# smann95/mpmc

Hardware: AMD Instinct MI355X
Metric: MC steps/sec (polarizable, 4096 atoms) (higher is better)
Workload: dtype f64; 1 GPU; PCN-61 cell + 416 BSSP H2, 4096 atoms (2016 frozen), polarizable, Jacobi x4, rc 8 A, FH4; energy() incremental (bit-identical to full); n_atoms=4096, n_polarizable=3264, n_atoms_final=4096, n_polarizable_final=3264, walkers=1, parallelism=1 independent walkers, 1 per GPU, collective=none (single walker, no launcher), rccl_ranks=1

## Files before the change

### include/mpmc_hip.h

```cpp
#ifndef MPMC_HIP_H
#define MPMC_HIP_H

#include <stddef.h>
#include <stdint.h>

#ifdef __cplusplus
extern "C" {
#endif

#define MPMC_HIP_ABI_VERSION 1

typedef struct mpmc_hip_ctx mpmc_hip_ctx;
typedef struct mpmc_hip_comm mpmc_hip_comm;

typedef struct mpmc_hip_params {
    double temperature;
    int rd_only;
    int rd_lrc;
    int feynman_hibbs;
    int feynman_hibbs_order;
    int ewald_alpha_set;
    double ewald_alpha;
    int ewald_kmax;
    int polarization;
    double polar_damp;
    int polar_max_iter;
    double polar_precision;
    double polar_gamma;
    int polar_gs;
    int polar_gs_ranked;
    int polar_sor;
    int polar_esor;
    int polar_palmo;
    int polar_rrms;
    int polar_zodid;
    int polar_wolf;
    double polar_wolf_alpha;
    int polar_ewald;
    int polar_ewald_alpha_set;
    double polar_ewald_alpha;
    int wolf;
} mpmc_hip_params;

typedef struct mpmc_hip_result {
    double energy;
    double rd_energy;
    double coulombic_energy;
    double polarization_energy;
    double es_real, es_recip, es_self;
    double dipole_rrms;
    double volume, cutoff, ewald_alpha, polar_ewald_alpha;
    int polar_iterations;
    int iter_success;
    int n_atoms;
    int status;
} mpmc_hip_result;

typedef struct mpmc_hip_timings {
    float pair_ms;
    float recip_ms;
    float field_ms;
    float amatrix_ms;
    float sweep_ms;
    float palmo_ms;
    float other_ms;
    float total_ms;
    int sweep_count;
    int amatrix_count;
    int graph_steps;
    float event_pair_ms;
    int event_pair_count;
    int spec_rank_redos;
    int resident_calls;
    int resident_fallbacks;
} mpmc_hip_timings;

const char *mpmc_hip_last_error(void);
int mpmc_hip_abi_version(void);
int mpmc_hip_device_count(void);

int mpmc_hip_create(mpmc_hip_ctx **ctx, int device, int max_atoms);
void mpmc_hip_destroy(mpmc_hip_ctx *ctx);

int mpmc_hip_set_option(mpmc_hip_ctx *ctx, const char *name, int value);

void mpmc_hip_default_params(mpmc_hip_params *p);
int mpmc_hip_set_params(mpmc_hip_ctx *ctx, const mpmc_hip_params *p);

int mpmc_hip_set_box(mpmc_hip_ctx *ctx, const double basis[9], double pbc_cutoff);

int mpmc_hip_scale_box(mpmc_hip_ctx *ctx, const double basis[9], double pbc_cutoff,
                       int n_molecules, const double *delta );

int mpmc_hip_upload(mpmc_hip_ctx *ctx, int n, const double *x, const double *y, const double *z,
                    const double *charge, const double *polarizability, const double *epsilon,
                    const double *sigma, const double *mass, const int *molecule, const uint8_t *frozen);

typedef struct mpmc_hip_disp_params {
    int disp_expansion;
    int damp_dispersion;
    int extrapolate_disp_coeffs;
    int schmidt_mixing;
} mpmc_hip_disp_params;

int mpmc_hip_set_dispersion(mpmc_hip_ctx *ctx, const mpmc_hip_disp_params *p, int n, const double *c6, const double *c8,
                            const double *c10);

int mpmc_hip_set_axilrod_teller(mpmc_hip_ctx *ctx, int enable, int n, const double *c9);
int mpmc_hip_get_three_body_energy(mpmc_hip_ctx *ctx, double *out);

int mpmc_hip_set_rd_crystal(mpmc_hip_ctx *ctx, int order);

int mpmc_hip_update_atoms(mpmc_hip_ctx *ctx, int first, int count, const double *x, const double *y,
                          const double *z);

int mpmc_hip_insert_molecule(mpmc_hip_ctx *ctx, int count, const double *x, const double *y, const double *z,
                             const double *charge, const double *polarizability, const double *epsilon,
                             const double *sigma, const double *mass, int frozen, int *first_slot);
int mpmc_hip_remove_molecule(mpmc_hip_ctx *ctx, int first_slot, int count);
int mpmc_hip_set_sweep_order(mpmc_hip_ctx *ctx, int count, const int *slots);
int mpmc_hip_slot_count(mpmc_hip_ctx *ctx);

int mpmc_hip_energy(mpmc_hip_ctx *ctx, mpmc_hip_result *out);

int mpmc_hip_energy_begin(mpmc_hip_ctx *ctx);
int mpmc_hip_energy_end(mpmc_hip_ctx *ctx, mpmc_hip_result *out);

// ... 25 lines not shown
```

### mpmc_amd/csrc/engine.hip

```cpp
#include "../../include/mpmc_hip.h"

#include <dlfcn.h>
#include <hip/hip_runtime.h>
#include <hip/hip_ext.h>
#include <rccl/rccl.h>

#include <algorithm>
#include <cmath>
#include <cstdarg>
#include <cstdio>
#include <cstring>
#include <functional>
#include <memory>
#include <tuple>
#include <utility>
#include <ctime>
#include <numeric>
#include <atomic>
#include <string>
#include <vector>

#include "device_common.h"
#include "kernels_pair.h"
#include "kernels_disp.h"
// ... 116 lines not shown
    R_RECIP = 5,
    R_SELF = 6,
    R_UPOL = 7,
    R_RRMS = 8,
    R_GS_ERR = 9,
    R_RMIN = 10,
    R_RANKCHG = 11,
    R_DISP = 12,
    R_DISP_LRC = 13,
    R_AT = 14,
    R_RDC_SELF = 15,
    R_COUNT = 16
};

struct SweepView {
    int nv = 0, nvpad = 0, cap = 0;
    DevBuf<int> d_idx;
    DevBuf<double> px, py, pz, palpha;
    DevBuf<int> pflags;
    DevBuf<double> A;
    bool A_valid = false;
    DevBuf<double2> C;
    int ntld = 0;
    DevBuf<double> energy_part;
    bool C_valid = false;
    bool pos_valid = false;
    unsigned long long ranked_call = 0;
    DevBuf<int> d_slot;
    std::vector<int> slot_of_atom;
    DevBuf<double> mupub;
    DevBuf<double> es, mu0, mu1, munew, y, efind, efchg, rrms;
    DevBuf<double> tmu0;
    DevBuf<unsigned> gsflags;
    DevBuf<double> Minv;
    DevBuf<double> Lnb[kGsMaxLag];
    int Lnb_lags = 0;
    int nlag = 0, nlag_built = 0;
    long long last_full_call = -1;
    int full_streak = 0;
    unsigned long long C_epoch = 0;
    unsigned long long M_epoch = 0;
    unsigned long long M_call = 0;
    int rebuild_from = -1;
    DevBuf<double> Srow;
    double *Zcol = nullptr;
    DevBuf<double> resP;
    int res_pld = 0;
    bool resP_armed = false;
    DevBuf<double> respub;
    std::vector<int> h_idx;
};

struct PendingSweep {
    bool on = false;
    struct SweepView *view = nullptr;
    const double *mu_in = nullptr;
    double *mu_out = nullptr;
    DevBox bx;
    SweepParams sp;
};

enum GraphSlotId { GS_MOVES = 0, GS_COEF, GS_FIELD, GS_PAIR, GS_RECIP, GS_PUBLISH, GS_NSLOT };
enum GraphMode { GM_DIRECT = 0, GM_CAPTURE = 1, GM_UPDATE = 2 };
struct StepGraph {
    hipGraph_t graph = nullptr;
    hipGraphExec_t exec = nullptr;
    void *func[GS_NSLOT] = {nullptr, nullptr, nullptr, nullptr, nullptr, nullptr};
    hipGraphNode_t node[GS_NSLOT] = {nullptr, nullptr, nullptr, nullptr, nullptr, nullptr};
    bool valid = false;
    unsigned long long rev = 0;
    int iterations = 0;
    struct SweepView *result_view = nullptr;
    const double *result_mu = nullptr;
    PendingSweep psweep;
    const double *energy_part = nullptr;
    int energy_nt = 0;
    int recip_chunks = 0, pair_rows_to_sum = 0;
    unsigned res_zero_mask = 0;
};

struct EngineOptions {
    int pair_coef = 1;
    int incremental = 1;
    int incremental_pairs = 1;
    int overlap = 1;
    int side_after = 1;
    int symmetric = 1;
    int sym_mode = 0;
    int timing = 1;
    int timing_interval = 32;
    int persistent_gs = 1;
    int spec_rank = 1;
    int fuse_tensor = 1;
    int gs_lags = 3;
    int gs_build_fork = 1;
    int gs_side_waves = 0;
    int rank_view_side = 1;
    int gs_fold_upper = 1;
    int gs_fold_finish = 1;
    int rank_late = 1;
    int resident = 1;
    int res_fold = 16;
    int res_side = 0;
    int sweep_alternate = 1;
    int sweep_nt = -1;
    int sweep_split = -1;
    int fuse_moves = 1;
    int gs_fuse_moves = 1;
    int fuse_field = 1;
    int fuse_recip = 1;
    int split_record = 1;
    int side_moves = 1;
// ... 177 lines not shown
    HipEvent ev_first, ev_last;
    bool timed = false;
    double host_enqueue_s = 0.0, host_wait_s = 0.0;
};

static DevAtoms dev_atoms(const mpmc_hip_ctx *c) {
    DevAtoms a;
    a.x = c->d_x;
    a.y = c->d_y;
    a.z = c->d_z;
    a.q = c->d_q;
    a.alpha = c->d_alpha;
    a.eps = (c->disp_on || c->rdc_order) ? c->d_zero : c->d_eps;
    a.sig = (c->disp_on || c->rdc_order) ? c->d_zero : c->d_sig;
    a.molmass = c->d_molmass;
    a.mol = c->d_mol;
    a.flags = c->d_flags;
    a.n = c->n;
    a.npad = c->npad;
    return a;
}

static DevBox dev_box(const mpmc_hip_ctx *c) {
    DevBox b;
    for (int p = 0; p < 3; ++p)
        for (int q = 0; q < 3; ++q) {
            b.b[p][q] = c->basis[p][q];
            b.rb[p][q] = c->recip[p][q];
        }
    b.cutoff = c->cutoff;
    b.volume = c->volume;
    for (int p = 0; p < 3; ++p)
        for (int q = 0; q < 3; ++q) {
            b.fb[p][q] = (float)c->basis[p][q];
            b.frb[p][q] = (float)c->recip[p][q];
        }
    b.rc2_pre = (float)((c->cutoff + 0.01) * (c->cutoff + 0.01));
    b.screen64 = (c->coord_max > kScreen32MaxCoord || !(c->coord_max == c->coord_max)) ? 1 : 0;
    double smax = 0.0, rmax = 0.0;
    for (int q = 0; q < 3; ++q) {
        smax = std::max(smax, std::fabs(c->recip[0][q]) + std::fabs(c->recip[1][q]) + std::fabs(c->recip[2][q]));
        for (int p = 0; p < 3; ++p) rmax = std::max(rmax, std::fabs(c->recip[p][q]));
    }
    const float tie32 = (float)(1.25 * 11.0 * 0x1p-13 * smax);
    b.half_tie32 = 0.5f - tie32;
    b.tie64 = 0x1p-49 * rmax;
    b.tie_guard = c->box_ortho ? 0 : 1;
    return b;
}

static int round_up(int v, int m) { return (v + m - 1) / m * m; }
static int complete_pending_sweep(mpmc_hip_ctx *c);
static void drop_polar_result(mpmc_hip_ctx *c) {
    c->psweep.on = false;
    c->have_polar_result = false;
}
static void (*chain_kernel_of(int ortho))(GsChain);

static void note_coords(mpmc_hip_ctx *c, const double *x, const double *y, const double *z, int count) {
    double m = c->coord_max;
    for (int i = 0; i < count; ++i) {
        const double v = std::max(std::fabs(x[i]), std::max(std::fabs(y[i]), std::fabs(z[i])));
        if (!(v <= m)) m = (v == v) ? v : INFINITY;
    }
    const bool was64 = c->coord_max > kScreen32MaxCoord;
    c->coord_max = m;
    if ((m > kScreen32MaxCoord) != was64) ++c->config_rev;
}

static inline bool is_timed_call(const mpmc_hip_ctx *c) {
    return c->opt.timing >= 2 || ((c->opt.timing == 1 || c->opt.timing == -1) &&
                                 (c->energy_calls % (unsigned long long)c->opt.timing_interval) == 0ull);
}

template <typename... KArgs, typename... Args, size_t... I>
static hipError_t launch_slot_impl(mpmc_hip_ctx *c, int slot, void (*kernel)(KArgs...), dim3 g, dim3 b, hipStream_t s,
                                   std::index_sequence<I...>, Args &&...args) {
    std::tuple<KArgs...> vals(std::forward<Args>(args)...);
    void *argv[] = {(void *)&std::get<I>(vals)...};
    if (c->graph_mode == GM_UPDATE) {
        hipKernelNodeParams p;
        memset(&p, 0, sizeof(p));
        p.func = (void *)kernel;
        p.gridDim = g;
        p.blockDim = b;
        p.sharedMemBytes = 0;
        p.kernelParams = argv;
        p.extra = nullptr;
        return hipGraphExecKernelNodeSetParams(c->sg.exec, c->sg.node[slot], &p);
    }
    c->sg.func[slot] = (void *)kernel;
    return hipLaunchKernel((const void *)kernel, g, b, argv, 0, s);
}
template <typename... KArgs, typename... Args>
static hipError_t launch_slot(mpmc_hip_ctx *c, int slot, void (*kernel)(KArgs...), dim3 g, dim3 b, hipStream_t s,
                              Args &&...args) {
    static_assert(sizeof...(KArgs) == sizeof...(Args), "argument count");
    return launch_slot_impl(c, slot, kernel, g, b, s, std::index_sequence_for<KArgs...>{}, std::forward<Args>(args)...);
}

struct ScopedTimer {
    mpmc_hip_ctx *c;
    hipStream_t s;
    TimeRec r;
    bool on;
    ScopedTimer(mpmc_hip_ctx *ctx, int cls, hipStream_t st = nullptr) : c(ctx), s(st ? st : ctx->stream), on(false) {
        const bool wanted = c->graph_mode == GM_DIRECT &&
// ... 1441 lines not shown
    const AtAtoms ta = {c->d_at_a, c->d_at_g};
    const long units = at_unit_count(ntile);
    return tile_pass(c, c->at, (int)(units * kAtSplit), R_AT, sb, [&](const DirtyBlocks &sel) {
        const dim3 grid = sel.n > 0 ? dim3((unsigned)(ntile * (ntile + 1) / 2 * kAtSplit), (unsigned)sel.n)
                                    : dim3((unsigned)(units * kAtSplit));
        hipLaunchKernelGGL(at_triple_kernel, grid, dim3(64 * kAtWaves), 0, sb, a, ta, bx, sel, ntile, c->at.part,
                           c->call.pair_moves);
    });
}

static int launch_publish(mpmc_hip_ctx *c) {
    const bool do_polar = c->call.do_polar;
    HIPCHK(launch_slot(c, GS_PUBLISH, publish_result_kernel, dim3(1), dim3(c->call.pair_rows_to_sum > 0 ? kReduceThreads : 64),
                       c->stream, c->d_res, c->h_res_dev,
                       (int)R_COUNT, (double)c->energy_calls, do_polar ? c->energy_part : (const double *)nullptr,
                       do_polar ? c->energy_nt : 0, c->n_valid,
                       c->call.gs_used[0] ? (const unsigned *)(c->view[0].gsflags + 1) : (const unsigned *)nullptr,
                       c->call.gs_used[1] ? (const unsigned *)(c->view[1].gsflags + 1) : (const unsigned *)nullptr,
                       (const double *)c->d_recipsum, c->call.split ? 0 : c->call.recip_chunks, c->call.res_zero_mask,
                       (const double *)c->d_pairpart, c->call.pair_rows_to_sum, (int)R_RD_PAIR, c->call.split ? kSideSlots : 0u));
    return 0;
}

static bool blocks_of(const std::vector<int> &atoms, DirtyBlocks &out) {
    memset(&out, 0, sizeof(out));
    for (int atom : atoms) {
        const int b = atom / 64;
        bool seen = false;
        for (int k = 0; k < out.n; ++k) seen |= (out.blk[k] == b);
        if (seen) continue;
        if (out.n == kMaxDirtyBlocks) {
            memset(&out, 0, sizeof(out));
            return false;
        }
        out.blk[out.n++] = b;
    }
    return true;
}

static void collect_dirty_blocks(mpmc_hip_ctx *c) {
    DirtyBlocks &d = c->call.dirty_blocks;
    if (c->all_dirty || !c->opt.incremental_pairs || !blocks_of(c->dirty_atoms, d)) {
        positions_unknown(c);
        memset(&d, 0, sizeof(d));
    }
    c->call.pair_part_valid_before = c->pair_part_valid;
}

static void begin_call(mpmc_hip_ctx *c) {
    ++c->energy_calls;
    c->ev_next = 0;
    c->recs.clear();
    c->call = CallState();
    c->psweep.on = false;
    collect_dirty_blocks(c);
}

static int enqueue_direct(mpmc_hip_ctx *c) {
    const mpmc_hip_params &P = c->par;
    CallState &k = c->call;
    k.do_polar = !P.rd_only && P.polarization;
    k.gs_mode = P.polar_gs || P.polar_gs_ranked;
    k.two_streams = c->opt.overlap && k.do_polar;
    k.plain_launches = c->graph_mode == GM_DIRECT && !c->opt.graph;
    const bool do_polar = k.do_polar, two_streams = k.two_streams;
    k.moves_deferred = c->opt.fuse_moves && c->pending.n > 0 && k.plain_launches && do_polar && !P.polar_zodid &&
                       (!k.gs_mode || (c->opt.gs_fuse_moves && gs_order_mode(c))) && P.polar_precision == 0.0 && c->opt.overlap &&
                       c->opt.pair_coef && !c->all_dirty && c->view[0].C_valid && c->view[0].pos_valid;
    k.moves_in_pair = !k.moves_deferred && c->opt.fuse_moves && c->pending.n > 0 && k.plain_launches && !do_polar &&
                      !c->dirty_atoms.empty();
    if (!k.moves_deferred && !k.moves_in_pair) {
        if (c->opt.side_moves && !c->main_writes && c->pending.n > 0 && two_streams && k.plain_launches)
            k.side_apply = c->pending;
        if (flush_moves(c)) return -1;
    } else if (k.moves_deferred && k.gs_mode) {
        if (c->opt.side_moves && !c->main_writes) k.side_apply = c->pending;
    }
    k.side_carry = k.moves_deferred && !k.gs_mode && c->opt.side_moves && !c->main_writes && !c->dirty_atoms.empty() &&
                   c->pending.n <= kMaxMoves;
    if (is_timed_call(c)) hipEventRecord(c->ev_first, c->stream);

    const DevAtoms a = dev_atoms(c);
    const DevBox bx = dev_box(c);
    const int ntile = c->npad / 64;
    int polar_iterations = 0, iter_success = 0;

    hipStream_t sb = two_streams ? c->stream2 : c->stream;
    k.split = two_streams && c->opt.split_record && !k.gs_mode && k.plain_launches;
    if (two_streams && !k.moves_deferred && k.side_apply.n == 0)
        hipEventRecord(c->ev_fork, c->stream);
    const bool polar_first = do_polar && two_streams && P.polar_precision == 0.0;
    int side_rc = 0;
    bool side_done = false;
    auto enqueue_side = [&]() {
        if (side_done) return;
        side_done = true;
        side_rc = [&]() -> int {
        if (two_streams && !(k.side_carry && k.side_moves.n > 0)) side_wait_for_moves(c, sb);
        if (P.rd_lrc) {
            DirtyBlocks lsel;
            const bool overflow = !blocks_of(c->lrc_dirty_atoms, lsel);
            if (!c->lrc.valid) lsel.n = 0;
            if (static_pass(c, c->lrc, !c->lrc.valid || overflow || lsel.n > 0, ntile * ntile, R_LRC, sb, [&] {
                    hipLaunchKernelGGL(lj_lrc_kernel, dim3(ntile, lsel.n > 0 ? lsel.n : ntile), dim3(64 * kLrcWaves), 0, sb, a, bx,
                                       lsel, c->lrc.part);
                }))
                return -1;
// ... 387 lines not shown
        SweepView *V = c->result_view;
        hipLaunchKernelGGL(scatter_results_kernel, dim3((c->npad + 255) / 256), dim3(256), 0, c->stream, c->npad,
                           V->d_slot, c->result_mu, V->efind, V->efchg, c->d_mu, c->d_efind, c->d_efchg);
        HIPCHK(hipStreamSynchronize(c->stream));
        c->results_scattered = true;
    }
    const size_t b = 3 * (size_t)c->n * sizeof(double);
    if (mu) HIPCHK(hipMemcpy(mu, c->d_mu, b, hipMemcpyDeviceToHost));
    if (ef_static) HIPCHK(hipMemcpy(ef_static, c->d_es, b, hipMemcpyDeviceToHost));
    if (ef_induced) HIPCHK(hipMemcpy(ef_induced, c->d_efind, b, hipMemcpyDeviceToHost));
    if (ef_induced_change) HIPCHK(hipMemcpy(ef_induced_change, c->d_efchg, b, hipMemcpyDeviceToHost));
    return 0;
}

extern "C" int mpmc_hip_download_amatrix(mpmc_hip_ctx *c, double *A) {
    if (!c || !c->have_atoms || !c->have_box || !A) return fail("MPMC_HIP: download_amatrix: no configuration");
    HIPCHK(hipSetDevice(c->device));
    const size_t n3 = 3 * (size_t)c->n, lda = 3 * (size_t)c->npad;
    if (flush_moves(c)) return -1;
    DevBuf<double> dA;
    HIPCHK(dA.alloc(lda * lda));
    hipLaunchKernelGGL(build_amatrix_kernel, dim3(c->npad / 128, c->npad / kARows), dim3(64), 0, c->stream,
                       dev_atoms(c), dev_box(c), c->par.polar_damp, dA, (int)lda);
    hipError_t e = hipMemcpy2DAsync(A, n3 * sizeof(double), dA, lda * sizeof(double), n3 * sizeof(double), n3,
                                    hipMemcpyDeviceToHost, c->stream);
    if (e == hipSuccess) e = hipStreamSynchronize(c->stream);
    if (e != hipSuccess) return fail("MPMC_HIP: download_amatrix: %s", hipGetErrorString(e));
    return 0;
}

extern "C" int mpmc_hip_download_ranking(mpmc_hip_ctx *c, double *rank_metric, int *ranked_array) {
    if (!c || !c->have_atoms) return fail("MPMC_HIP: download_ranking: no configuration");
    HIPCHK(hipSetDevice(c->device));
    if (rank_metric) HIPCHK(hipMemcpy(rank_metric, c->d_rank, c->n * sizeof(double), hipMemcpyDeviceToHost));
    if (ranked_array) {
        std::vector<int> perm(c->n);
        std::iota(perm.begin(), perm.end(), 0);
        if (c->perm_ranked && (int)c->rank_saved.size() == c->n) {
            const double *rk = c->rank_saved.data();
            std::stable_sort(perm.begin(), perm.end(), [rk](int x, int y) { return rk[x] > rk[y]; });
        }
        memcpy(ranked_array, perm.data(), c->n * sizeof(int));
    }
    return 0;
}

extern "C" int mpmc_hip_get_timings(mpmc_hip_ctx *c, mpmc_hip_timings *t) {
    if (!c || !t) return fail("MPMC_HIP: get_timings: null argument");
    memset(t, 0, sizeof(*t));
    t->graph_steps = (int)c->graph_launches;
    t->spec_rank_redos = (int)c->spec_redos;
    t->resident_calls = (int)c->resident_calls;
    t->resident_fallbacks = (int)c->resident_fallbacks;
    if (!c->timed) return 0;
    HIPCHK(hipSetDevice(c->device));
    float acc[T_NCLASS] = {0};
    int cnt[T_NCLASS] = {0};
    for (const TimeRec &r : c->recs) {
        float ms = 0.f;
        HIPCHK(hipEventSynchronize(r.b));
        HIPCHK(hipEventElapsedTime(&ms, r.a, r.b));
        acc[r.cls] += ms;
        cnt[r.cls]++;
    }
    t->pair_ms = acc[T_PAIR];
    t->recip_ms = acc[T_RECIP];
    t->field_ms = acc[T_FIELD];
    t->amatrix_ms = acc[T_AMAT];
    t->sweep_ms = acc[T_SWEEP];
    t->palmo_ms = acc[T_PALMO];
    t->other_ms = acc[T_OTHER];
    t->sweep_count = cnt[T_SWEEP];
    t->amatrix_count = cnt[T_AMAT];
    t->event_pair_ms = acc[T_EVPAIR];
    t->event_pair_count = cnt[T_EVPAIR];
    float tot = 0.f;
    HIPCHK(hipEventElapsedTime(&tot, c->ev_first, c->ev_last));
    t->total_ms = tot;
    return 0;
}

struct Rccl {
    void *h = nullptr;
    ncclResult_t (*GetUniqueId)(ncclUniqueId *) = nullptr;
    ncclResult_t (*CommInitRank)(ncclComm_t *, int, ncclUniqueId, int) = nullptr;
    ncclResult_t (*AllReduce)(const void *, void *, size_t, ncclDataType_t, ncclRedOp_t, ncclComm_t,
                              hipStream_t) = nullptr;
    ncclResult_t (*AllGather)(const void *, void *, size_t, ncclDataType_t, ncclComm_t, hipStream_t) = nullptr;
    ncclResult_t (*CommDestroy)(ncclComm_t) = nullptr;
    const char *(*GetErrorString)(ncclResult_t) = nullptr;
};
static Rccl g_rccl;

struct mpmc_hip_comm {
    HipStream stream;
    ncclComm_t nccl = nullptr;
    int device = 0;
    DevBuf<double> d_buf;
    PinnedBuf<double> h_buf;
    int nranks = 1, rank = 0;
    int pending = 0;
    DevBuf<unsigned char> d_gather;
    PinnedBuf<unsigned char> h_gather;
    ~mpmc_hip_comm() {
        if (stream) hipStreamSynchronize(stream);
        if (nccl) g_rccl.CommDestroy(nccl);
// ... 115 lines not shown
```

### mpmc_amd/csrc/engine_polar.inc

```
static constexpr bool kSweepSplitAuto = false;

static int launch_coef_job(mpmc_hip_ctx *c, const DevBox &bx) {
    if (!c->call.coef_job_valid) return 0;
    c->call.coef_job_valid = false;
    const CoefJob &cj = c->call.coef_job;
    hipLaunchKernelGGL(update_coef_moves_kernel, dim3(cj.nt, cj.dm.n), dim3(64), 0, c->stream, cj.pa, bx, cj.damp, cj.dm,
                       cj.ntld, cj.C, cj.m, cj.gx, cj.gy, cj.gz, cj.slot_of_atom, cj.px, cj.py, cj.pz);
    if (c->call.coef_job_fork) hipEventRecord(c->ev_fork, c->stream);
    return 0;
}

static int launch_field(mpmc_hip_ctx *c, const DevAtoms &a, const DevBox &bx) {
    const mpmc_hip_params &P = c->par;
    ScopedTimer t(c, T_FIELD);
    FieldParams fp;
    fp.wolf_alpha = P.polar_wolf_alpha;
    fp.cutoffterm = 0.0;
    const int ntile = c->npad / 64;
    int nchunk = std::max(1, std::min(ntile, 4096 / ntile));
    int chunk = round_up((c->npad + nchunk - 1) / nchunk, 64);
    nchunk = (c->npad + chunk - 1) / chunk;
    fp.chunk = chunk;
    const int mode = P.polar_ewald ? kFieldEwald : (!P.polar_wolf ? kFieldBare : (P.polar_wolf_alpha == 0.0 ? kFieldWolf0 : kFieldWolfA));
    const int key = mode * 1000003 + chunk;
// ... 383 lines not shown
                                    : (sweep_nt ? pair_sweep_kernel<0, 1, 0, 1> : pair_sweep_kernel<0, 0, 0, 1>);
            if (c->opt.sweep_ablate == 1) kern = pair_sweep_kernel<1, 0, 1>;
            if (c->opt.sweep_ablate == 2) kern = pair_sweep_kernel<1, 0, 2>;
            if (c->opt.sweep_ablate) half_plane = 0;
            HIPCHK(launch_timed(c, timer_class, kern, g, b, 0, c->stream, (const double2 *)v.C, nt, v.ntld,
                                (const double *)v.px, (const double *)v.py, (const double *)v.pz, mu_in, bx, v.Srow, v.Zcol,
                                c->opt.sweep_alternate ? (c->sweep_parity++ & 1) : 0, half_plane));
        }
        {
            ScopedTimer t2(c, T_OTHER);
            hipLaunchKernelGGL(pair_finish_kernel<MODE>, dim3(nt), dim3(64 * kCoefFinishGroups), 0, c->stream, nt, v.Srow,
                               v.Zcol, fin, half_plane);
        }
        c->energy_part = v.energy_part;
        c->energy_nt = nt;
        return 0;
    }
    c->energy_nt = 0;
    if (c->opt.symmetric && (nvpad >= 2048 || c->opt.symmetric > 1)) {
        if (ensure_sym_scratch(v)) return -1;
        {
            ScopedTimer t(c, timer_class);
            const dim3 g(nvpad / kSymChunkAtoms, nvpad / kSymRowAtoms);
            const int rev = (c->opt.sym_mode & 1) ? (c->sweep_parity++ & 1) : 0;
            if (c->opt.sym_mode & 2)
                hipLaunchKernelGGL(symv_kernel<1>, g, dim3(64), 0, c->stream, v.A, lda, nvpad, mu_in, v.Srow, v.Zcol, rev,
                                   v.nv);
            else
                hipLaunchKernelGGL(symv_kernel<0>, g, dim3(64), 0, c->stream, v.A, lda, nvpad, mu_in, v.Srow, v.Zcol, rev,
                                   v.nv);
        }
        ScopedTimer t2(c, T_OTHER);
        hipLaunchKernelGGL(symv_finish_kernel<MODE>, dim3(nvpad / 64), dim3(1024), 0, c->stream, nvpad, v.Srow, v.Zcol,
                           v.palpha, v.pflags, mu_in, v.es, v.efind, out, v.rrms, c->d_errmax, sp);
    } else {
        ScopedTimer t(c, timer_class);
        hipLaunchKernelGGL(sweep_kernel<MODE>, dim3(nvpad), dim3(64), 0, c->stream, v.A, lda, nvpad, v.palpha,
                           v.pflags, mu_in, v.es, v.efind, out, v.rrms, c->d_errmax, sp);
    }
    return 0;
}

static bool defer_last_sweep(const mpmc_hip_ctx *c, const SweepView &v) {
    const mpmc_hip_params &P = c->par;
    if (!c->opt.pair_coef || !v.C_valid) return false;
    if (P.polar_zodid || P.polar_gs || P.polar_gs_ranked || P.polar_palmo || P.polar_sor || P.polar_esor || P.polar_rrms)
        return false;
    if (P.polar_precision != 0.0 || P.polar_gamma != 1.0 || P.polar_max_iter < 2) return false;
    const int nt = std::max(1, (v.nv + kCoefTile - 1) / kCoefTile);
    return nt * (nt + 1) / 2 + nt > c->num_cus;
}

static int complete_pending_sweep(mpmc_hip_ctx *c) {
    if (!c->psweep.on) return 0;
    const PendingSweep p = c->psweep;
    c->psweep.on = false;
    HIPCHK(hipSetDevice(c->device));
    return launch_sweep<kSweepJacobi>(c, *p.view, p.bx, p.mu_in, p.mu_out, p.sp, T_SWEEP);
}

static void (*chain_kernel_of(int ortho))(GsChain) { return ortho ? gs_chain_kernel<1> : gs_chain_kernel<0>; }

static bool gs_uses_chain(const mpmc_hip_ctx *c) { return c->opt.pair_coef != 0 && c->opt.persistent_gs != 0; }

struct GsFinishArgs {
    double w_new, w_old;
    int want_rrms, err_slot;
    double *mu_out;
};
static int launch_gs_sweep(mpmc_hip_ctx *c, SweepView &v, const DevAtoms &a, const DevBox &bx, const double *mu_old,
                           const GsFinishArgs *fin = nullptr, bool *finished = nullptr) {
    if (finished) *finished = false;
    const int nvpad = v.nvpad, lda = 3 * nvpad;
    (void)a;
    ++c->call.gs_sweeps;
    if (gs_uses_chain(c) && v.C_valid) {
        const int nt = std::max(1, (v.nv + kCoefTile - 1) / kCoefTile);
        if (ensure_coef_scratch(v, nt)) return -1;
        const bool fold_upper = c->opt.gs_fold_upper && fin && c->opt.gs_fold_finish && !c->opt.gs_ablate;
        {
            ScopedTimer tu(c, T_OTHER);
            const dim3 g(nt * (nt + 1) / 2), b(64 * kCoefWaves);
            const int rev = c->opt.sweep_alternate ? (c->sweep_parity++ & 1) : 0;
            if (c->box_ortho)
                hipLaunchKernelGGL(pair_upper_kernel<1>, g, b, 0, c->stream, v.C, nt, v.ntld, v.px, v.py, v.pz, mu_old, bx, v.Srow, rev,
                                   fold_upper ? nt : 0, v.mupub, v.gsflags, c->gs_qoff);
            else
                hipLaunchKernelGGL(pair_upper_kernel<0>, g, b, 0, c->stream, v.C, nt, v.ntld, v.px, v.py, v.pz, mu_old, bx, v.Srow, rev,
                                   fold_upper ? nt : 0, v.mupub, v.gsflags, c->gs_qoff);
            if (!fold_upper)
                hipLaunchKernelGGL(pair_upper_finish_kernel, dim3(nvpad / 64), dim3(64 * kCoefFinishGroups), 0, c->stream, nt,
                                   v.Srow, v.y, 1, v.mupub, v.gsflags, c->gs_qoff);
        }
        GsChain gp;
        gp.C = v.C;
        gp.ntld = v.ntld;
        gp.nb = nt;
        gp.px = v.px;
        gp.py = v.py;
        gp.pz = v.pz;
        gp.alpha = v.palpha;
        gp.es = v.es;
        gp.Minv = v.Minv;
        for (int k = 0; k < kGsMaxLag; ++k) {
            gp.Lnb[k] = v.Lnb[k];
            gp.pub[k] = v.mupub + k * (size_t)c->gs_qoff;
        }
        gp.nlag = v.nlag >= 2 ? v.nlag : c->opt.gs_lags;
        gp.y = v.y;
        gp.mu_new = v.mupub;
        gp.flags = v.gsflags;
// ... 230 lines not shown
        if (spec_rank) {
            if (rank_side) side_wait_for_moves(c, rs);
            W.ranked_call = c->energy_calls;
            if (setup_view(c, W, a, bx, true, true, false, true, rs)) return -1;
            hipEventRecord(c->ev_rank, rs);
            enqueue_rank_metric();
        } else if (rank_side) {
            enqueue_rank_metric();
            HIPCHK(hipMemcpyAsync(c->h_rank, c->d_rank, n * sizeof(double), hipMemcpyDeviceToHost, rs));
            hipEventRecord(c->ev_rank, rs);
        } else {
            enqueue_rank_metric();
        }
        c->call.rank_on_side = rank_side && !spec_rank;
        return 0;
        }();
    };
    if (!(c->opt.rank_late && spec_rank)) {
        enqueue_rank();
        if (rank_rc) return -1;
    }

    SweepView *V = &c->view[0];
    if (!P.polar_zodid) {
        const bool chain = gs && gs_uses_chain(c);
        if (setup_view(c, *V, a, bx, true, c->opt.pair_coef != 0, (gs && !chain) || !c->opt.pair_coef, chain)) return -1;
    } else {
        const dim3 g((V->nvpad + 255) / 256), b(256);
        hipLaunchKernelGGL(gather_atoms_kernel, g, b, 0, c->stream, V->nv, V->nvpad, V->d_idx, a, V->px, V->py, V->pz,
                           V->palpha, V->pflags);
    }

    if (ranked && spec_rank && c->opt.rank_late >= 2) enqueue_rank_metric();

    if (launch_field(c, a, bx)) return -1;

    double *mu_in = V->mu0, *mu_out = V->mu1;
    const ResidentPlan rp = resident_plan(c, *V);
    if (rp.ok && ensure_view_resident(c, *V)) return -1;
    c->call.resident = rp.ok;
    {
        const double scale = (!P.polar_sor && !P.polar_esor) ? P.polar_gamma : 1.0;
        hipLaunchKernelGGL(init_view_kernel, dim3(V->nvpad / 64), dim3(64 * kFieldGroups), 0, c->stream, V->nv,
                           V->nvpad, V->d_idx, V->palpha, c->d_fieldpart, c->es_slots, c->npad, scale, V->es, mu_in,
                           V->efind, V->efchg, V->rrms, c->d_errmax,
                           (chain_mode || rp.ok) ? c->view[0].gsflags : (unsigned *)nullptr,
                           chain_mode ? c->view[1].gsflags : (unsigned *)nullptr,
                           rp.ok ? V->respub : (double *)nullptr, P.polar_max_iter, (size_t)3 * V->nvpad);
    }

    int iteration_counter = 0;
    bool ranked_active = false;
    const bool defer = !rp.ok && defer_last_sweep(c, *V);
    if (rp.ok) {
        if (launch_resident(c, *V, bx, rp, want_rrms)) return -1;
        iteration_counter = P.polar_max_iter;
        mu_in = V->mu1;
    } else if (!P.polar_zodid) {
        bool keep_iterating = true;
        while (keep_iterating) {
            iteration_counter++;
            const int nvpad = V->nvpad;
            const dim3 gvec((nvpad + 255) / 256), bvec(256);
            if (iteration_counter >= kMAX_ITERATION_COUNT && P.polar_precision != 0.0) {
                hipLaunchKernelGGL(fallback_dipoles_kernel, gvec, bvec, 0, c->stream, nvpad, V->palpha, V->es, mu_in,
                                   V->efchg);
                *iter_success = 1;
                break;
            }
            double w_new = 1.0, w_old = 0.0;
            if (P.polar_sor) {
                w_new = P.polar_gamma;
                w_old = 1.0 - P.polar_gamma;
            } else if (P.polar_esor) {
                w_old = std::exp(-P.polar_gamma * iteration_counter);
                w_new = 1.0 - w_old;
            }
            const double *palmo_mu = mu_in;
            if (!gs) {
                SweepParams sp;
                sp.w_new = w_new;
                sp.w_old = w_old;
                sp.want_rrms = want_rrms;
                sp.want_err = P.polar_precision > 0.0;
                sp.err_slot = iteration_counter;
                sp.skip_sums = (P.polar_precision == 0.0 && iteration_counter < P.polar_max_iter) ? 1 : 0;
                const int mid = (P.polar_max_iter + 1) / 2;
                if (defer) {
                    const bool odd = P.polar_max_iter & 1;
                    sp.skip_sums = 1;
                    if (odd && iteration_counter == P.polar_max_iter - mid) sp.energy_mode |= kEnergyStoreSums;
                    if (iteration_counter == mid) sp.energy_mode |= kEnergyMid | (odd ? kEnergyPrevSums : 0);
                }
                if (defer && iteration_counter == P.polar_max_iter) {
                    sp.skip_sums = 1;
                    PendingSweep &ps = c->psweep;
                    ps.on = true;
                    ps.view = V;
                    ps.mu_in = mu_in;
                    ps.mu_out = mu_out;
                    ps.bx = bx;
                    ps.sp = sp;
                } else if (launch_sweep<kSweepJacobi>(c, *V, bx, mu_in, mu_out, sp, T_SWEEP)) {
                    return -1;
                }
                if (c->call.enqueue_side && (iteration_counter == c->opt.side_after || P.polar_max_iter < c->opt.side_after)) c->call.enqueue_side();
                if (defer && iteration_counter == mid && c->call.publish_early) {
                    if (c->call.enqueue_side) c->call.enqueue_side();
                    c->call.publish_early();
                }
            } else {
                GsFinishArgs gfa;
                gfa.w_new = w_new;
                gfa.w_old = w_old;
                gfa.want_rrms = (int)want_rrms;
                gfa.err_slot = (P.polar_precision > 0.0) ? iteration_counter : -1;
                gfa.mu_out = mu_out;
                bool finished = false;
                if (launch_gs_sweep(c, *V, a, bx, mu_in, &gfa, &finished)) return -1;
                const bool planar = gs_uses_chain(c) && V->C_valid;
                if (!finished)
                hipLaunchKernelGGL(gs_finish_kernel, gvec, bvec, 0, c->stream, nvpad, V->palpha, V->pflags, mu_in,
                                   (const double *)(planar ? V->mupub : V->munew), planar ? 1 : 0, V->y, w_new, w_old,
                                   (int)want_rrms, iteration_counter, mu_out, planar ? V->munew : (double *)nullptr,
                                   V->efind, V->rrms, c->d_errmax);
                palmo_mu = V->munew;
            }

            if (P.polar_precision == 0.0) {
                keep_iterating = (iteration_counter != P.polar_max_iter);
            } else {
                HIPCHK(hipMemcpyAsync(c->h_err, c->d_errmax + iteration_counter, sizeof(unsigned long long),
                                      hipMemcpyDeviceToHost, c->stream));
                HIPCHK(hipStreamSynchronize(c->stream));
                double emax;
                memcpy(&emax, c->h_err, sizeof(double));
                const double allowed = P.polar_precision * P.polar_precision * kDEBYE2SKA * kDEBYE2SKA;
                keep_iterating = (emax > allowed);
            }

            if (P.polar_palmo && !keep_iterating) {
                SweepParams sp;
                sp.w_new = 1.0;
                sp.w_old = 0.0;
                sp.want_rrms = 0;
                sp.want_err = 0;
                sp.err_slot = 0;
                sp.skip_sums = 0;
                if (launch_sweep<kSweepPalmo>(c, *V, bx, palmo_mu, V->efchg, sp, T_PALMO, gs ? V->munew : mu_out)) return -1;
            }

            std::swap(mu_in, mu_out);

            if (ranked && !rank_enqueued) {
                enqueue_rank();
// ... 104 lines not shown
```

### mpmc_amd/engine.py

```python
import ctypes as C
import os

import numpy as np

_HERE = os.path.dirname(os.path.abspath(__file__))
LIB_PATH = os.path.join(_HERE, "csrc", "libmpmc_hip.so")

EXPORTS = [
    "mpmc_hip_last_error", "mpmc_hip_abi_version", "mpmc_hip_device_count", "mpmc_hip_create",
    "mpmc_hip_destroy", "mpmc_hip_set_option", "mpmc_hip_default_params", "mpmc_hip_set_params", "mpmc_hip_set_box",
    "mpmc_hip_scale_box",
    "mpmc_hip_upload", "mpmc_hip_set_dispersion", "mpmc_hip_set_axilrod_teller", "mpmc_hip_get_three_body_energy",
    "mpmc_hip_set_rd_crystal",
    "mpmc_hip_update_atoms", "mpmc_hip_insert_molecule", "mpmc_hip_remove_molecule",
    "mpmc_hip_slot_count", "mpmc_hip_set_sweep_order", "mpmc_hip_energy", "mpmc_hip_energy_begin", "mpmc_hip_energy_end",
    "mpmc_hip_download_dipoles",
    "mpmc_hip_download_amatrix", "mpmc_hip_download_ranking", "mpmc_hip_get_timings",
    "mpmc_hip_comm_unique_id", "mpmc_hip_comm_create", "mpmc_hip_comm_size", "mpmc_hip_comm_rank",
    "mpmc_hip_allreduce_observables", "mpmc_hip_allreduce_observables_begin", "mpmc_hip_allreduce_observables_end",
    "mpmc_hip_gather_observables", "mpmc_hip_comm_destroy",
]


class Params(C.Structure):
# ... 16 lines not shown
        ("polar_sor", C.c_int),
        ("polar_esor", C.c_int),
        ("polar_palmo", C.c_int),
        ("polar_rrms", C.c_int),
        ("polar_zodid", C.c_int),
        ("polar_wolf", C.c_int),
        ("polar_wolf_alpha", C.c_double),
        ("polar_ewald", C.c_int),
        ("polar_ewald_alpha_set", C.c_int),
        ("polar_ewald_alpha", C.c_double),
        ("wolf", C.c_int),
    ]


class Result(C.Structure):
    _fields_ = [
        ("energy", C.c_double),
        ("rd_energy", C.c_double),
        ("coulombic_energy", C.c_double),
        ("polarization_energy", C.c_double),
        ("es_real", C.c_double),
        ("es_recip", C.c_double),
        ("es_self", C.c_double),
        ("dipole_rrms", C.c_double),
        ("volume", C.c_double),
        ("cutoff", C.c_double),
        ("ewald_alpha", C.c_double),
        ("polar_ewald_alpha", C.c_double),
        ("polar_iterations", C.c_int),
        ("iter_success", C.c_int),
        ("n_atoms", C.c_int),
        ("status", C.c_int),
    ]


class Timings(C.Structure):
    _fields_ = [
        ("pair_ms", C.c_float),
        ("recip_ms", C.c_float),
        ("field_ms", C.c_float),
        ("amatrix_ms", C.c_float),
        ("sweep_ms", C.c_float),
        ("palmo_ms", C.c_float),
        ("other_ms", C.c_float),
        ("total_ms", C.c_float),
        ("sweep_count", C.c_int),
        ("amatrix_count", C.c_int),
        ("graph_steps", C.c_int),
        ("event_pair_ms", C.c_float),
        ("event_pair_count", C.c_int),
        ("spec_rank_redos", C.c_int),
        ("resident_calls", C.c_int),
        ("resident_fallbacks", C.c_int),
    ]


class DispParams(C.Structure):
    _fields_ = [
        ("disp_expansion", C.c_int),
        ("damp_dispersion", C.c_int),
        ("extrapolate_disp_coeffs", C.c_int),
        ("schmidt_mixing", C.c_int),
    ]


PARAM_NAMES = [f[0] for f in Params._fields_]
DISP_NAMES = [f[0] for f in DispParams._fields_]
AT_NAMES = ["axilrod_teller", "midzuno_kihara_approx"]
RDC_NAMES = ["rd_crystal", "rd_crystal_order"]
NOT_PARAMS = frozenset(["pbc_cutoff"] + DISP_NAMES + AT_NAMES + RDC_NAMES)
AT_ALPHA_AU = 6.7483345

_lib = None


def load():
    global _lib
    if _lib is not None:
        return _lib
    if not os.path.exists(LIB_PATH):
        raise RuntimeError(
            "libmpmc_hip.so is not built (run `python -c 'import __graft_entry__ as g; g.build()'`); "
            "there is no CPU fallback")
    lib = C.CDLL(LIB_PATH)
    dp = C.POINTER(C.c_double)
    vp = C.c_void_p
    lib.mpmc_hip_last_error.restype = C.c_char_p
    lib.mpmc_hip_abi_version.restype = C.c_int
    lib.mpmc_hip_device_count.restype = C.c_int
    lib.mpmc_hip_create.argtypes = [C.POINTER(vp), C.c_int, C.c_int]
    lib.mpmc_hip_destroy.argtypes = [vp]
    lib.mpmc_hip_destroy.restype = None
    lib.mpmc_hip_set_option.argtypes = [vp, C.c_char_p, C.c_int]
    lib.mpmc_hip_default_params.argtypes = [C.POINTER(Params)]
    lib.mpmc_hip_default_params.restype = None
    lib.mpmc_hip_set_params.argtypes = [vp, C.POINTER(Params)]
    lib.mpmc_hip_set_box.argtypes = [vp, dp, C.c_double]
    lib.mpmc_hip_scale_box.argtypes = [vp, dp, C.c_double, C.c_int, vp]
    lib.mpmc_hip_upload.argtypes = [vp, C.c_int] + [vp] * 10
    lib.mpmc_hip_set_dispersion.argtypes = [vp, C.POINTER(DispParams), C.c_int, vp, vp, vp]
    lib.mpmc_hip_set_axilrod_teller.argtypes = [vp, C.c_int, C.c_int, vp]
    lib.mpmc_hip_get_three_body_energy.argtypes = [vp, dp]
    lib.mpmc_hip_set_rd_crystal.argtypes = [vp, C.c_int]
    lib.mpmc_hip_update_atoms.argtypes = [vp, C.c_int, C.c_int, vp, vp, vp]
    lib.mpmc_hip_insert_molecule.argtypes = [vp, C.c_int, vp, vp, vp, vp, vp, vp, vp, vp, C.c_int, C.POINTER(C.c_int)]
    lib.mpmc_hip_remove_molecule.argtypes = [vp, C.c_int, C.c_int]
# ... 204 lines not shown
```

### mpmc_amd/host/energy_hip.c

```c
#include <math.h>
#include <stdint.h>
#include <stdio.h>
#include <stdlib.h>
#include <string.h>
#include <time.h>

#ifdef MPMC_SHIM_HOST_MIRROR
#include "mpmc_host.h"
#else
#include <structs.h>
#include <function_prototypes.h>
extern int rank, size;
#endif
#include "energy_hip.h"


typedef struct {
    molecule_t *mol;
    atom_t *atoms;
    int slot, natoms, frozen;
} resident_t;

typedef struct shim_state {
    system_t *system;
// ... 604 lines not shown
            }
            if (mpmc_hip_create(&st->ctx, device, st->capacity)) {
                hip_fail("create");
                return device_failed(st);
            }
            st->device = device;
            st->uploaded = 0;
        }
        if (full_upload(st, system)) return device_failed(st);
    }
    const double t1 = now_s();
    if (mpmc_hip_energy_begin(st->ctx)) {
        hip_fail("energy");
        return device_failed(st);
    }
    g_prof[0] += t1 - t0;
    g_prof[1] += now_s() - t1;
    return 0;
}

double energy_hip_end(system_t *system) {
    shim_state *st = state_of(system, 0);
    if (!st || !st->ctx) return NAN;
    const double t2 = now_s();
    update_com(system->molecules);
    countN(system);
    const double t3 = now_s();
    mpmc_hip_result r;
    if (mpmc_hip_energy_end(st->ctx, &r)) {
        hip_fail("energy");
        device_failed(st);
        return NAN;
    }
    const double t4 = now_s();
    g_prof[2] += t3 - t2; g_prof[3] += t4 - t3;
    if (++g_prof_calls == 64) {
        g_prof[0] = g_prof[1] = g_prof[2] = g_prof[3] = 0.0;
        g_prof_t0 = t4;
        g_prof_base = 64;
    }
    g_prof_tlast = t4;
    if (st->timing) {
        mpmc_hip_timings t;
        if (!mpmc_hip_get_timings(st->ctx, &t)) {
            mpmc_hip_timings *s = &st->tsum;
            s->pair_ms += t.pair_ms; s->recip_ms += t.recip_ms; s->field_ms += t.field_ms;
            s->amatrix_ms += t.amatrix_ms; s->sweep_ms += t.sweep_ms; s->palmo_ms += t.palmo_ms;
            s->other_ms += t.other_ms; s->total_ms += t.total_ms;
            s->sweep_count += t.sweep_count; s->amatrix_count += t.amatrix_count;
            s->event_pair_ms += t.event_pair_ms; s->event_pair_count += t.event_pair_count;
            s->spec_rank_redos = t.spec_rank_redos;
            s->resident_calls = t.resident_calls;
            s->resident_fallbacks = t.resident_fallbacks;
        }
    }
    observables_t *o = system->observables;
    o->rd_energy = r.rd_energy;
    o->coulombic_energy = r.coulombic_energy;
    o->polarization_energy = r.polarization_energy;
    o->energy = r.energy;
    o->three_body_energy = 0.0;
    if (system->axilrod_teller && mpmc_hip_get_three_body_energy(st->ctx, &o->three_body_energy)) {
        hip_fail("get_three_body_energy");
        device_failed(st);
        return NAN;
    }
    o->dipole_rrms = r.dipole_rrms;
    system->nodestats->polarization_iterations = (double)r.polar_iterations;
    if (r.iter_success) system->iter_success = 1;
    if (o->N > 0.0) o->spin_ratio /= o->N;
    o->NU = o->N * o->energy;
    system->last_volume = system->pbc->volume;
    return o->energy;
}

double energy_hip(system_t *system) {
    if (energy_hip_begin(system)) return NAN;
    return energy_hip_end(system);
}

int energy_hip_download_dipoles(system_t *system) {
    shim_state *st = state_of(system, 0);
    if (!st || !st->ctx) return -1;
    const int n = mpmc_hip_slot_count(st->ctx);
    double *buf = malloc(4 * 3 * (size_t)(n > 0 ? n : 1) * sizeof(double));
    if (!buf) return -1;
    double *mu = buf, *es = buf + 3 * n, *ei = buf + 6 * n, *ec = buf + 9 * n;
    if (mpmc_hip_download_dipoles(st->ctx, mu, es, ei, ec)) {
        free(buf);
        return hip_fail("download_dipoles");
    }
    int r = 0;
    for (molecule_t *m = system->molecules; m && r < st->nres; m = m->next, r++) {
        int i = st->res[r].slot;
        for (atom_t *a = m->atoms; a; a = a->next, i++)
            for (int p = 0; p < 3; p++) {
                a->mu[p] = mu[3 * i + p];
                a->ef_static[p] = es[3 * i + p];
                a->ef_induced[p] = ei[3 * i + p];
                a->ef_induced_change[p] = ec[3 * i + p];
            }
    }
    free(buf);
    return 0;
}

// ... 117 lines not shown
```

Baseline: 12230 MC steps/s.

## Defer multiple trailing Jacobi sweeps past energy publication

Changes the pending-sweep mechanism from a single deferred final Jacobi sweep to a list of sweeps. Once the energy has been published after the midpoint iteration, all remaining Jacobi sweeps are queued and launched later instead of inline. The aim is to take more sweep work off the critical path of the energy result. The final sweep no longer sets skip_sums, which may change what deferred sweeps compute, and a new pending_sweeps counter is exposed in the timings struct.

```diff
diff --git a/include/mpmc_hip.h b/include/mpmc_hip.h
--- a/include/mpmc_hip.h
+++ b/include/mpmc_hip.h
@@ -73,6 +73,7 @@
     int spec_rank_redos;
     int resident_calls;
     int resident_fallbacks;
+    int pending_sweeps;
 } mpmc_hip_timings;
 
 const char *mpmc_hip_last_error(void);
diff --git a/mpmc_amd/csrc/engine.hip b/mpmc_amd/csrc/engine.hip
--- a/mpmc_amd/csrc/engine.hip
+++ b/mpmc_amd/csrc/engine.hip
@@ -192,12 +192,15 @@
 };
 
 struct PendingSweep {
-    bool on = false;
+    struct One {
+        const double *mu_in = nullptr;
+        double *mu_out = nullptr;
+        SweepParams sp;
+    };
+    std::vector<One> sweeps;
     struct SweepView *view = nullptr;
-    const double *mu_in = nullptr;
-    double *mu_out = nullptr;
     DevBox bx;
-    SweepParams sp;
+    void drop() { sweeps.clear(); }
 };
 
 enum GraphSlotId { GS_MOVES = 0, GS_COEF, GS_FIELD, GS_PAIR, GS_RECIP, GS_PUBLISH, GS_NSLOT };
@@ -481,7 +484,7 @@
 static int round_up(int v, int m) { return (v + m - 1) / m * m; }
 static int complete_pending_sweep(mpmc_hip_ctx *c);
 static void drop_polar_result(mpmc_hip_ctx *c) {
-    c->psweep.on = false;
+    c->psweep.drop();
     c->have_polar_result = false;
 }
 static void (*chain_kernel_of(int ortho))(GsChain);
@@ -2029,7 +2032,7 @@
     c->ev_next = 0;
     c->recs.clear();
     c->call = CallState();
-    c->psweep.on = false;
+    c->psweep.drop();
     collect_dirty_blocks(c);
 }
 
@@ -2523,6 +2526,7 @@
     t->spec_rank_redos = (int)c->spec_redos;
     t->resident_calls = (int)c->resident_calls;
     t->resident_fallbacks = (int)c->resident_fallbacks;
+    t->pending_sweeps = (int)c->psweep.sweeps.size();
     if (!c->timed) return 0;
     HIPCHK(hipSetDevice(c->device));
     float acc[T_NCLASS] = {0};
diff --git a/mpmc_amd/csrc/engine_polar.inc b/mpmc_amd/csrc/engine_polar.inc
--- a/mpmc_amd/csrc/engine_polar.inc
+++ b/mpmc_amd/csrc/engine_polar.inc
@@ -459,11 +459,13 @@
 }
 
 static int complete_pending_sweep(mpmc_hip_ctx *c) {
-    if (!c->psweep.on) return 0;
-    const PendingSweep p = c->psweep;
-    c->psweep.on = false;
+    if (c->psweep.sweeps.empty()) return 0;
+    PendingSweep p;
+    std::swap(p, c->psweep);
     HIPCHK(hipSetDevice(c->device));
-    return launch_sweep<kSweepJacobi>(c, *p.view, p.bx, p.mu_in, p.mu_out, p.sp, T_SWEEP);
+    for (const PendingSweep::One &s : p.sweeps)
+        if (launch_sweep<kSweepJacobi>(c, *p.view, p.bx, s.mu_in, s.mu_out, s.sp, T_SWEEP)) return -1;
+    return 0;
 }
 
 static void (*chain_kernel_of(int ortho))(GsChain) { return ortho ? gs_chain_kernel<1> : gs_chain_kernel<0>; }
@@ -800,6 +802,7 @@
     int iteration_counter = 0;
     bool ranked_active = false;
     const bool defer = !rp.ok && defer_last_sweep(c, *V);
+    c->psweep.drop();
     if (rp.ok) {
         if (launch_resident(c, *V, bx, rp, want_rrms)) return -1;
         iteration_counter = P.polar_max_iter;
@@ -840,15 +843,15 @@
                     if (odd && iteration_counter == P.polar_max_iter - mid) sp.energy_mode |= kEnergyStoreSums;
                     if (iteration_counter == mid) sp.energy_mode |= kEnergyMid | (odd ? kEnergyPrevSums : 0);
                 }
-                if (defer && iteration_counter == P.polar_max_iter) {
-                    sp.skip_sums = 1;
+                if (defer && (iteration_counter == P.polar_max_iter || (iteration_counter > mid && c->call.published))) {
                     PendingSweep &ps = c->psweep;
-                    ps.on = true;
                     ps.view = V;
-                    ps.mu_in = mu_in;
-                    ps.mu_out = mu_out;
                     ps.bx = bx;
-                    ps.sp = sp;
+                    PendingSweep::One one;
+                    one.mu_in = mu_in;
+                    one.mu_out = mu_out;
+                    one.sp = sp;
+                    ps.sweeps.push_back(one);
                 } else if (launch_sweep<kSweepJacobi>(c, *V, bx, mu_in, mu_out, sp, T_SWEEP)) {
                     return -1;
                 }
diff --git a/mpmc_amd/engine.py b/mpmc_amd/engine.py
--- a/mpmc_amd/engine.py
+++ b/mpmc_amd/engine.py
@@ -92,6 +92,7 @@
         ("spec_rank_redos", C.c_int),
         ("resident_calls", C.c_int),
         ("resident_fallbacks", C.c_int),
+        ("pending_sweeps", C.c_int),
     ]
 
 
diff --git a/mpmc_amd/host/energy_hip.c b/mpmc_amd/host/energy_hip.c
--- a/mpmc_amd/host/energy_hip.c
+++ b/mpmc_amd/host/energy_hip.c
@@ -680,6 +680,7 @@
             s->spec_rank_redos = t.spec_rank_redos;
             s->resident_calls = t.resident_calls;
             s->resident_fallbacks = t.resident_fallbacks;
+            s->pending_sweeps = t.pending_sweeps;
         }
     }
     observables_t *o = system->observables;
```

New measurement: 13850 MC steps/s (median of 6 runs). 1.13x the previous value.
